# jaxsonpd/air_rs

Hardware: AMD Instinct MI355X
Metric: IQ Msamples/s (decoded Mode-S msgs/s alongside), 2 MSPS i8 stream (higher is better)
Workload: dtype i8; 1 GPU; 2 MSPS i8 IQ, 1 GiB synthetic buffer per GPU, fused magnitude+preamble/DF17 gate+PPM+CRC-24; samples_per_gpu=536870912, bytes_per_gpu=1073741824, channels=1

## Files before the change

air_rs_amd/csrc/adsb_kernels.hip:

```cpp
#include <hip/hip_ext.h>
#include <utility>
#include <cstdlib>

#include "adsb_kernels.h"
#include "adsb_synth.h"

namespace adsbk {

typedef unsigned int u32x4 __attribute__((ext_vector_type(4)));
typedef unsigned short u16x2 __attribute__((ext_vector_type(2)));

__device__ __forceinline__ uint32_t pkmin(uint32_t a, uint32_t b)
{
    u16x2 r = __builtin_elementwise_min(__builtin_bit_cast(u16x2, a), __builtin_bit_cast(u16x2, b));
    return __builtin_bit_cast(uint32_t, r);
}
__device__ __forceinline__ uint32_t pkmax(uint32_t a, uint32_t b)
{
    u16x2 r = __builtin_elementwise_max(__builtin_bit_cast(u16x2, a), __builtin_bit_cast(u16x2, b));
    return __builtin_bit_cast(uint32_t, r);
}
typedef _Float16 f16x2 __attribute__((ext_vector_type(2)));
template <bool F16> __device__ __forceinline__ uint32_t pkmax3(uint32_t a, uint32_t b, uint32_t c)
{
// ... 65 lines not shown
    float f[8];
#pragma unroll
    for (int k = 0; k < 4; k += 2) {
        f32x2 ta = {__builtin_bit_cast(float, a[k]), __builtin_bit_cast(float, a[k + 1])};
        f32x2 tb = {__builtin_bit_cast(float, b[k]), __builtin_bit_cast(float, b[k + 1])};
        f32x2 te = ta - (f32x2){8388607.5f, 8388607.5f};
        f32x2 to = __builtin_elementwise_fma(ta, (f32x2){-0x1.fffffep-1f, -0x1.fffffep-1f}, tb);
        f[2 * k] = te.x;
        f[2 * k + 1] = to.x;
        f[2 * k + 2] = te.y;
        f[2 * k + 3] = to.y;
    }
    float r[8];
#pragma unroll
    for (int k = 0; k < 8; ++k) {
        r[k] = __builtin_amdgcn_sqrtf(f[k]);
        if (MAGMODE == 2) r[k] -= 0.5f;
    }
    lo = __builtin_amdgcn_cvt_pk_u8_f32(r[0], 0, 0u);
    lo = __builtin_amdgcn_cvt_pk_u8_f32(r[1], 1, lo);
    lo = __builtin_amdgcn_cvt_pk_u8_f32(r[2], 2, lo);
    lo = __builtin_amdgcn_cvt_pk_u8_f32(r[3], 3, lo);
    hi = __builtin_amdgcn_cvt_pk_u8_f32(r[4], 0, 0u);
    hi = __builtin_amdgcn_cvt_pk_u8_f32(r[5], 1, hi);
    hi = __builtin_amdgcn_cvt_pk_u8_f32(r[6], 2, hi);
    hi = __builtin_amdgcn_cvt_pk_u8_f32(r[7], 3, hi);
}

__device__ __forceinline__ uint32_t mag_i16_fix(uint32_t r, uint32_t n)
{
    return r - ((__umul24(r, r) > n) ? 1u : 0u);
}
__device__ __forceinline__ uint32_t mag_i16(uint32_t iq)
{
    uint32_t n, r;
    asm("v_dot2_i32_i16 %0, %2, %2, 0\n\t"
        "s_nop 2\n\t"
        "v_cvt_f32_u32 %1, %0\n\t"
        "v_sqrt_f32 %1, %1\n\t"
        "s_nop 0\n\t"
        "v_cvt_rpi_i32_f32 %1, %1"
        : "=&v"(n), "=&v"(r)
        : "v"(iq));
    return mag_i16_fix(r, n);
}
__device__ __forceinline__ void mags4_i16(u32x4 v, uint32_t &lo, uint32_t &hi)
{
    uint32_t n0, n1, n2, n3, r0, r1, r2, r3;
    asm("v_dot2_i32_i16 %0, %8, %8, 0\n\t"
        "v_dot2_i32_i16 %1, %9, %9, 0\n\t"
        "v_dot2_i32_i16 %2, %10, %10, 0\n\t"
        "v_dot2_i32_i16 %3, %11, %11, 0\n\t"
        "s_nop 2\n\t"
        "v_cvt_f32_u32 %4, %0\n\t"
        "v_cvt_f32_u32 %5, %1\n\t"
        "v_cvt_f32_u32 %6, %2\n\t"
        "v_cvt_f32_u32 %7, %3\n\t"
        "v_sqrt_f32 %4, %4\n\t"
        "v_sqrt_f32 %5, %5\n\t"
        "v_sqrt_f32 %6, %6\n\t"
        "v_sqrt_f32 %7, %7\n\t"
        "v_cvt_rpi_i32_f32 %4, %4\n\t"
        "v_cvt_rpi_i32_f32 %5, %5\n\t"
        "v_cvt_rpi_i32_f32 %6, %6\n\t"
        "s_nop 0\n\t"
        "v_cvt_rpi_i32_f32 %7, %7\n\t"
        "s_nop 0"
        : "=&v"(n0), "=&v"(n1), "=&v"(n2), "=&v"(n3), "=&v"(r0), "=&v"(r1), "=&v"(r2), "=&v"(r3)
        : "v"(v.x), "v"(v.y), "v"(v.z), "v"(v.w));
    lo = __builtin_amdgcn_perm(mag_i16_fix(r1, n1), mag_i16_fix(r0, n0), 0x05040100u);
    hi = __builtin_amdgcn_perm(mag_i16_fix(r3, n3), mag_i16_fix(r2, n2), 0x05040100u);
}

__global__ void probe_cvt_kernel(uint32_t *out)
{
    if (threadIdx.x != 0) return;
    float a = 0.75f, b = 2.5f, c = 180.9986f;
    asm volatile("" : "+v"(a), "+v"(b), "+v"(c));
    uint32_t r0 = __builtin_amdgcn_cvt_pk_u8_f32(a, 0, 0u);
    r0 = __builtin_amdgcn_cvt_pk_u8_f32(b, 1, r0);
    r0 = __builtin_amdgcn_cvt_pk_u8_f32(c, 2, r0);
    out[0] = r0;
    __builtin_amdgcn_s_setreg((1 | (0 << 6) | ((2 - 1) << 11)), 3);
    asm volatile("" : "+v"(a), "+v"(b), "+v"(c));
    uint32_t r1 = __builtin_amdgcn_cvt_pk_u8_f32(a, 0, 0u);
    r1 = __builtin_amdgcn_cvt_pk_u8_f32(b, 1, r1);
    r1 = __builtin_amdgcn_cvt_pk_u8_f32(c, 2, r1);
    out[1] = r1;
    __builtin_amdgcn_s_setreg((1 | (0 << 6) | ((2 - 1) << 11)), 0);
    out[2] = 0xC0DEu;
    out[3] = 0;
}

hipError_t probe_cvt(hipStream_t s, uint32_t *dev_scratch4, uint32_t host_out[4])
{
    hipLaunchKernelGGL(probe_cvt_kernel, dim3(1), dim3(64), 0, s, dev_scratch4);
    hipError_t e = hipGetLastError();
    if (e != hipSuccess) return e;
    e = hipMemcpyAsync(host_out, dev_scratch4, 16, hipMemcpyDeviceToHost, s);
    if (e != hipSuccess) return e;
    return hipStreamSynchronize(s);
}

template <int ST> struct MagT;
template <> struct MagT<ADSB_SAMPLE_I8> { typedef uint8_t type; };
template <> struct MagT<ADSB_SAMPLE_I16> { typedef uint16_t type; };

template <int ST> struct Lds {
    typedef typename MagT<ST>::type mag_t;
    static constexpr int kMagBytes = (TileCfg<ST>::kMagT * (int)sizeof(mag_t) + 15) & ~15;
    static constexpr int kOffCand = kMagBytes;
    static constexpr int kOffList = kOffCand + 2 * kThreads * 4 * ((TileCfg<ST>::kRunT + 31) / 32);
    static constexpr int kOffMisc = kOffList + kListCap * 2;
    static constexpr int kTotal = kOffMisc + 64;
};

template <int ST>
__device__ __forceinline__ uint32_t pair_at(const uint32_t *ra, const uint32_t *rb, int k)
{
    if (ST == ADSB_SAMPLE_I8) {
        const uint32_t sel = 0x0C000C00u | (uint32_t)(k & 3) | ((uint32_t)(4 + (k & 3)) << 16);
        return __builtin_amdgcn_perm(rb[k >> 2], ra[k >> 2], sel);
    } else {
        const uint32_t sel = (k & 1) ? 0x07060302u : 0x05040100u;
        return __builtin_amdgcn_perm(rb[k >> 1], ra[k >> 1], sel);
    }
}

template <int ST>
__device__ __forceinline__ uint32_t pair_at_cold(const uint32_t *ra, const uint32_t *rb, int k)
{
    if (ST == ADSB_SAMPLE_I8) {
        const uint32_t sel = 0x0C000C00u | (uint32_t)(4 + (k & 3)) | ((uint32_t)(k & 3) << 16);
        return __builtin_amdgcn_perm(ra[k >> 2], rb[k >> 2], sel);
    } else {
        const uint32_t sel = (k & 1) ? 0x03020706u : 0x01000504u;
        return __builtin_amdgcn_perm(ra[k >> 1], rb[k >> 1], sel);
    }
}

#define ADSB_DPP(v, ctrl) ((uint32_t)__builtin_amdgcn_update_dpp(0, (int)(v), (ctrl), 0xF, 0xF, true))
__device__ __forceinline__ uint32_t row16_xor(uint32_t v)
{
    v ^= ADSB_DPP(v, 0xB1);
    v ^= ADSB_DPP(v, 0x4E);
    v ^= ADSB_DPP(v, 0x141);
    v ^= ADSB_DPP(v, 0x140);
    return v;
}

template <int ST>
__device__ __forceinline__ uint32_t slice_byte(const typename MagT<ST>::type *mag, const uint32_t off, const uint32_t lb)
{
    uint32_t byte = 0;
    if (ST == ADSB_SAMPLE_I16) {
        const typename MagT<ST>::type *mp = mag + off + 16 + 16 * lb;
#pragma unroll
        for (int k = 0; k < 8; ++k)
            byte |= (((uint32_t)mp[2 * k + 1] - (uint32_t)mp[2 * k]) >> 31) << (7 - k);
    } else {
        const uint32_t pidx = off + 16 + 16 * lb;
        const uint32_t *mw = reinterpret_cast<const uint32_t *>(mag) + (pidx >> 2);
        const uint32_t sh = pidx & 3;
        const uint32_t d0 = mw[0], d1 = mw[1], d2 = mw[2], d3 = mw[3], d4 = mw[4];
        uint32_t w[4] = {__builtin_amdgcn_alignbyte(d1, d0, sh), __builtin_amdgcn_alignbyte(d2, d1, sh),
                         __builtin_amdgcn_alignbyte(d3, d2, sh), __builtin_amdgcn_alignbyte(d4, d3, sh)};
        uint64_t m0, m1, m2, m3, m4, m5, m6, m7;
        asm("v_cmp_gt_u32_sdwa %1, %9, %9 src0_sel:BYTE_0 src1_sel:BYTE_1\n\t"
            "v_cmp_gt_u32_sdwa %2, %9, %9 src0_sel:BYTE_2 src1_sel:BYTE_3\n\t"
            "v_cmp_gt_u32_sdwa %3, %10, %10 src0_sel:BYTE_0 src1_sel:BYTE_1\n\t"
            "v_cmp_gt_u32_sdwa %4, %10, %10 src0_sel:BYTE_2 src1_sel:BYTE_3\n\t"
            "v_cmp_gt_u32_sdwa %5, %11, %11 src0_sel:BYTE_0 src1_sel:BYTE_1\n\t"
            "v_cmp_gt_u32_sdwa %6, %11, %11 src0_sel:BYTE_2 src1_sel:BYTE_3\n\t"
            "v_cmp_gt_u32_sdwa %7, %12, %12 src0_sel:BYTE_0 src1_sel:BYTE_1\n\t"
            "v_cmp_gt_u32_sdwa %8, %12, %12 src0_sel:BYTE_2 src1_sel:BYTE_3\n\t"
            "v_addc_co_u32_e64 %0, vcc, %0, %0, %1\n\t"
            "v_addc_co_u32_e64 %0, vcc, %0, %0, %2\n\t"
            "v_addc_co_u32_e64 %0, vcc, %0, %0, %3\n\t"
            "v_addc_co_u32_e64 %0, vcc, %0, %0, %4\n\t"
            "v_addc_co_u32_e64 %0, vcc, %0, %0, %5\n\t"
            "v_addc_co_u32_e64 %0, vcc, %0, %0, %6\n\t"
            "v_addc_co_u32_e64 %0, vcc, %0, %0, %7\n\t"
            "v_addc_co_u32_e64 %0, vcc, %0, %0, %8"
            : "+v"(byte), "=&s"(m0), "=&s"(m1), "=&s"(m2), "=&s"(m3), "=&s"(m4), "=&s"(m5), "=&s"(m6), "=&s"(m7)
            : "v"(w[0]), "v"(w[1]), "v"(w[2]), "v"(w[3])
            : "vcc");
    }
    return byte;
}

__device__ __forceinline__ bool count_candidate(const bool have, const uint32_t byte, const uint32_t l, const uint32_t lane)
{
    const uint32_t lb = l < 14 ? l : 13;
    uint32_t s = 0;
    const uint32_t *sy = kSyn.v + 8 * lb;
    const int sb = (int)(l < 14 ? byte : 0u);
#pragma unroll
    for (int k = 0; k < 8; ++k) s ^= sy[k] & (uint32_t)((sb << (24 + k)) >> 31);
    s = row16_xor(s);
    int found = -1;
    if (s != 0 && l < 11) {
#pragma unroll
        for (int k = 0; k < 8; ++k) found = (sy[k] == s) ? k : found;
    }
    const unsigned long long fm = __ballot(found >= 0);
    const uint32_t gbits = (uint32_t)(fm >> (lane & 48u)) & 0xFFFFu;
    return have && (s == 0 || gbits != 0);
}

struct TilePos {
    uint32_t ch;
    uint64_t sample0;
    uint32_t n_valid;
};
template <int TILE = kTile>
__device__ __forceinline__ TilePos tile_pos(const DemodArgs &p, uint32_t tile)
{
    TilePos t;
    t.ch = tile / p.tiles_per_channel;
    const uint32_t tch = tile - t.ch * p.tiles_per_channel;
    t.sample0 = (uint64_t)tch * TILE;
    const uint64_t left = (p.n_samples - kWindow) - t.sample0;
    t.n_valid = left < (uint64_t)TILE ? (uint32_t)left : (uint32_t)TILE;
    return t;
}

template <int BPS, int MAG = kMag>
__device__ __forceinline__ __amdgpu_buffer_rsrc_t tile_rsrc(const DemodArgs &p, const TilePos &t, bool live = true)
{
    const char *base = (const char *)p.iq + ((uint64_t)t.ch * p.channel_stride + t.sample0) * BPS;
    const uint64_t remain = (p.n_samples - t.sample0) * BPS;
    const uint32_t nrec = remain > (uint64_t)(MAG * BPS) ? (uint32_t)(MAG * BPS) : (uint32_t)remain;
    return __builtin_amdgcn_make_buffer_rsrc((void *)base, 0, live ? (int)nrec : 0, 0x00020000);
}

#ifndef ADSB_TILE_STAMPS
#define ADSB_TILE_STAMPS 0
#endif
#if ADSB_TILE_STAMPS
#define TSTAMP(k)                                                                                              \
    do {                                                                                                       \
        if ((tid & 63u) == 0 && (wave == 0 || wave == 3)) {                                                    \
            __builtin_amdgcn_sched_barrier(0);                                                                 \
            const unsigned long long now_ = __builtin_amdgcn_s_memtime();                                      \
            if ((k) >= 0) ts_seg[(k)] = (uint32_t)(now_ - ts_prev);                                            \
            ts_prev = now_;                                                                                    \
            __builtin_amdgcn_sched_barrier(0);                                                                 \
        }                                                                                                      \
    } while (0)
#else
#define TSTAMP(k) do { } while (0)
#endif

#ifndef ADSB_AB_KERNELS
#define ADSB_AB_KERNELS 0
#endif
bool ab_kernels_built() { return ADSB_AB_KERNELS != 0; }

template <int RUN, int NT>
__device__ __forceinline__ void gate_collect(uint32_t *candA, uint32_t *candB, uint16_t *list, uint32_t *count,
                                             const uint32_t tid, const uint32_t n_valid)
{
    constexpr int WPR = (RUN + 31) / 32;
    const uint32_t sa = tid * RUN, sb = (tid + NT) * RUN;
    const uint32_t va = n_valid > sa ? (n_valid - sa) : 0u, vb = n_valid > sb ? (n_valid - sb) : 0u;
    uint32_t words[2 * WPR];
    uint32_t nz = 0, c = 0;
#pragma unroll
    for (int k = 0; k < WPR; ++k) {
        words[k] = candA[k];
        words[WPR + k] = candB[k];
    }
    if (n_valid < (uint32_t)(2 * NT * RUN)) {
#pragma unroll
        for (int k = 0; k < WPR; ++k) {
            const uint32_t la = va > 32u * k ? va - 32u * k : 0u, lb = vb > 32u * k ? vb - 32u * k : 0u;
            words[k] &= la >= 32u ? 0xFFFFFFFFu : ((1u << la) - 1u);
            words[WPR + k] &= lb >= 32u ? 0xFFFFFFFFu : ((1u << lb) - 1u);
            candA[k] = words[k];
            candB[k] = words[WPR + k];
        }
    }
#pragma unroll
    for (int k = 0; k < 2 * WPR; ++k) {
        nz |= words[k];
        c += __builtin_popcount(words[k]);
    }
    if (nz) {
        uint32_t pos = atomicAdd(count, c);
#pragma unroll
        for (int k = 0; k < 2 * WPR; ++k) {
            uint32_t bits = words[k];
            const uint32_t base = (k < WPR ? sa : sb) + (k % WPR) * 32;
            while (bits) {
                const uint32_t b = __builtin_ctz(bits);
                bits &= bits - 1;
                if (pos < (uint32_t)kSparseCap) list[pos] = (uint16_t)(base + b);
                ++pos;
            }
        }
    }
}

template <int ST, int RUN, int NT, bool F16OK = (ST == ADSB_SAMPLE_I8)>
__device__ __forceinline__ void gate_phase(const typename MagT<ST>::type *mag, uint32_t *cand, uint16_t *list,
                                           uint32_t *count, const uint32_t tid, const uint32_t n_valid)
{
    static_assert(RUN == 16 || RUN == 32 || RUN == 64, "1 or 2 bitmap words per run");
    constexpr int WPR = (RUN + 31) / 32;
    constexpr int SPG = 16 / (int)sizeof(typename MagT<ST>::type);
    uint32_t *candA = cand + WPR * tid, *candB = cand + WPR * (tid + NT);
#pragma unroll
    for (int k = 0; k < WPR; ++k) candA[k] = candB[k] = 0u;
    constexpr int kGran = (RUN + 26 + SPG - 1) / SPG + 1;
    const u32x4 *ga = reinterpret_cast<const u32x4 *>(mag + tid * RUN);
    const u32x4 *gb = reinterpret_cast<const u32x4 *>(mag + (tid + NT) * RUN);
    uint32_t ra[kGran * 4], rb[kGran * 4];
    constexpr int kAhead = 48 / SPG;
#pragma unroll
    for (int g = 0; g < kAhead; ++g) {
        u32x4 a = ga[g], b = gb[g];
        ra[4 * g] = a.x; ra[4 * g + 1] = a.y; ra[4 * g + 2] = a.z; ra[4 * g + 3] = a.w;
        rb[4 * g] = b.x; rb[4 * g + 1] = b.y; rb[4 * g + 2] = b.z; rb[4 * g + 3] = b.w;
    }

    uint32_t N[RUN + 26], H2[RUN + 8], W3[RUN + 16], F[RUN + 9];
#pragma unroll
    for (int k = 0; k < 25; ++k) N[k] = pair_at<ST>(ra, rb, k);
#pragma unroll
    for (int j = 0; j < 7; ++j) H2[j] = pkmin(N[j], N[j + 2]);
#pragma unroll
    for (int j = 3; j < 13; ++j) W3[j] = pkmax3<F16OK>(N[j], N[j + 1], N[j + 2]);
#pragma unroll
    for (int j = 1; j < 8; ++j) F[j] = pkmax3<F16OK>(N[j], W3[j + 2], N[j + 5]);

#pragma unroll
    for (int o = 0; o < RUN; ++o) {
        if (o % SPG == 0) {
            const int g = o / SPG + kAhead;
            if (g * SPG < RUN + 26) {
                u32x4 a = ga[g], b = gb[g];
                ra[4 * g] = a.x; ra[4 * g + 1] = a.y; ra[4 * g + 2] = a.z; ra[4 * g + 3] = a.w;
                rb[4 * g] = b.x; rb[4 * g + 1] = b.y; rb[4 * g + 2] = b.z; rb[4 * g + 3] = b.w;
            }
        }
        N[o + 25] = pair_at<ST>(ra, rb, o + 25);
        W3[o + 13] = pkmax3<F16OK>(N[o + 13], N[o + 14], N[o + 15]);
        F[o + 8] = pkmax3<F16OK>(N[o + 8], W3[o + 10], N[o + 13]);
        const uint32_t lo = pkmax3<F16OK>(F[o + 1], F[o + 8], W3[o + 13]);
        H2[o + 7] = pkmin(N[o + 7], N[o + 9]);
        const uint32_t hi = pkmin(H2[o], H2[o + 7]);
        const bool pa = (uint16_t)hi >= (uint16_t)lo;
        const bool pb = (hi >> 16) >= (lo >> 16);
        if (__builtin_expect(__builtin_amdgcn_ballot_w64(pa | pb) != 0, 0)) {
            const uint32_t dh = pkmin3<F16OK>(pkmin3<F16OK>(N[o + 16], N[o + 19], N[o + 21]), N[o + 23], N[o + 24]);
            const uint32_t dl = pkmax3<F16OK>(pkmax3<F16OK>(N[o + 17], N[o + 18], N[o + 20]), N[o + 22], N[o + 25]);
            const bool da = (uint16_t)dh >= (uint16_t)dl;
            const bool db = (dh >> 16) >= (dl >> 16);
            uint32_t bit = 1u << (o & 31);
            asm("" : "+v"(bit));
            if (pa & da) atomicOr(candA + (o >> 5), bit);
            if (pb & db) atomicOr(candB + (o >> 5), bit);
        }
    }
    gate_collect<RUN, NT>(candA, candB, list, count, tid, n_valid);
}

#ifndef ADSB_LOAD_AUX
#define ADSB_LOAD_AUX 2
#endif
template <int ST> struct P1 {
    static constexpr int kSPL = ST == ADSB_SAMPLE_I8 ? 8 : 4;
    static constexpr int kIters = (TileCfg<ST>::kMagT + kThreads * kSPL - 1) / (kThreads * kSPL);
};

template <int ST>
__device__ __forceinline__ void issue_tile_loads(const DemodArgs &p, const TilePos &tp, bool live, uint32_t tid,
                                                 u32x4 (&raw)[P1<ST>::kIters])
{
    constexpr int BPS = (ST == ADSB_SAMPLE_I8) ? 2 : 4;
    __amdgpu_buffer_rsrc_t rsrc = tile_rsrc<BPS, TileCfg<ST>::kMagT>(p, tp, live);
    const uint32_t wave_s0 = __builtin_amdgcn_readfirstlane(tid & ~63u) * P1<ST>::kSPL;
#pragma unroll
    for (int it = 0; it < P1<ST>::kIters; ++it)
        if ((uint32_t)it * (kThreads * P1<ST>::kSPL) + wave_s0 < (uint32_t)TileCfg<ST>::kMagT)
            raw[it] = __builtin_amdgcn_raw_buffer_load_b128(rsrc, tid * 16, (uint32_t)it * (kThreads * 16), ADSB_LOAD_AUX);
}

template <int ST, int MAGMODE>
__device__ __forceinline__ bool magnitudes_to_lds(const u32x4 (&raw)[P1<ST>::kIters], typename MagT<ST>::type *mag, uint32_t tid)
{
    uint32_t mx = 0;
    const uint32_t wave_s0 = __builtin_amdgcn_readfirstlane(tid & ~63u) * P1<ST>::kSPL;
#pragma unroll
    for (int it = 0; it < P1<ST>::kIters; ++it) {
        if ((uint32_t)it * (kThreads * P1<ST>::kSPL) + wave_s0 < (uint32_t)TileCfg<ST>::kMagT) {
            const uint32_t s = (uint32_t)it * (kThreads * P1<ST>::kSPL) + tid * P1<ST>::kSPL;
            uint32_t lo, hi;
            if (ST == ADSB_SAMPLE_I8) mags8_i8<MAGMODE>(raw[it], lo, hi);
            else {
                mags4_i16(raw[it], lo, hi);
                mx = pkmax(mx, pkmax(lo, hi));
            }
            if (s < (uint32_t)TileCfg<ST>::kMagT) *reinterpret_cast<uint2 *>(mag + s) = make_uint2(lo, hi);
        }
    }
    return ST == ADSB_SAMPLE_I16 && __builtin_amdgcn_ballot_w64(((mx & 0xFFFFu) >= 0x7C00u) || ((mx >> 16) >= 0x7C00u)) != 0;
}

__device__ __forceinline__ void clear_launch_flags(const DemodArgs &p, const bool first, const uint32_t tid)
{
    if (tid == 0 && first) {
        p.hdr->retry = 0;
        if (p.count_groups) {
            p.hdr->flags = 0;
            if (p.hdr_pub) p.hdr_pub[2] = 0;
        }
    }
}
__device__ __forceinline__ void tile_prologue(const DemodArgs &p, const bool first, uint32_t *misc, const uint32_t tid)
{
    clear_launch_flags(p, first, tid);
    if (tid == 0) {
        misc[8] = 0;
        misc[12] = 0;
    }
}


__device__ __forceinline__ void put_record(adsb_frame *slot, const uint64_t o64, const uint32_t byte, const uint32_t l)
{
    unsigned char *rec = reinterpret_cast<unsigned char *>(slot);
    if (l < 14) rec[8 + l] = (unsigned char)byte;
    else reinterpret_cast<uint32_t *>(rec)[l - 14] = l == 14 ? (uint32_t)o64 : (uint32_t)(o64 >> 32);
}

__device__ __forceinline__ void write_seg(const DemodArgs &p, const uint32_t tile, const uint32_t base_slot, const uint32_t cand,
                                          const uint32_t valid)
{
    Seg e;
    e.base = base_slot;
    e.cand = cand;
    e.valid = valid;
    e.decoded = base_slot == kNoBase ? 1u : 0u;
    p.seg[tile] = e;
}

constexpr uint32_t kCountBitmap = 0xFFFFFFFFu;
struct NoRecheck {
    __device__ __forceinline__ void operator()(uint16_t *, uint32_t) const {}
};
template <int TILE, int BITS, class SLICER, class RECHECK = NoRecheck>
__device__ __forceinline__ void hand_over(const DemodArgs &p, const uint32_t tile, const uint64_t sample0, uint32_t total,
                                          const uint32_t *cand, uint16_t *list, uint32_t *misc, const uint32_t tid,
                                          const uint32_t lane, const uint32_t wave, SLICER slicer, RECHECK recheck = RECHECK())
{
    const bool dense = total > (uint32_t)kSparseCap;
    u32x4 cw = {0, 0, 0, 0};
    uint32_t cnt = 0, my_first = 0;
    if (dense) {
        if (4 * tid < (uint32_t)(TILE / BITS)) cw = reinterpret_cast<const u32x4 *>(cand)[tid];
        cnt = __builtin_popcount(cw.x) + __builtin_popcount(cw.y) + __builtin_popcount(cw.z) +
              __builtin_popcount(cw.w);
        uint32_t incl = cnt;
#pragma unroll
        for (int d = 1; d < 64; d <<= 1) {
            uint32_t t = __shfl_up(incl, d, 64);
            if ((int)lane >= d) incl += t;
        }
        if (lane == 63) misc[wave] = incl;
        __syncthreads();
        uint32_t wbase = 0;
        total = 0;
#pragma unroll
        for (int w = 0; w < kThreads / 64; ++w) {
            uint32_t t = misc[w];
            wbase += (w < (int)wave) ? t : 0u;
            total += t;
        }
        my_first = wbase + incl - cnt;
    }

    const bool simple = !dense && total <= kQuota;
    const uint64_t abs0 = sample0 + p.offset_base;
    uint32_t base_slot = tile * kQuota;
    const uint32_t g = tid >> 4, l = tid & 15;
    auto slice_round = [&](uint32_t slot0, uint32_t ncl) {
        for (uint32_t r = 0; r < ncl; r += kThreads / 16) {
            if (r + 4 * wave >= ncl) break;
            const uint32_t ci = r + g;
            const bool have = ci < ncl;
            const uint32_t off = have ? list[ci] : 0u;
            bool dropped;
            const uint32_t byte = slicer(have, off, l, dropped);
            if (have) put_record(p.slots + (size_t)slot0 + ci, dropped ? ~0ull : abs0 + off, byte, l);
        }
    };
    if (simple) {
        slice_round(base_slot, total);
    } else {
        if (tid == 0) {
            const unsigned long long b64 = atomicAdd(&p.hdr->alloc, (unsigned long long)total);
            misc[9] = (!p.pool_off && b64 + total <= (unsigned long long)p.cap_slots) ? p.pool_first + (uint32_t)b64 : kNoBase;
        }
        __syncthreads();
        base_slot = misc[9];
        for (uint32_t chunk = 0; chunk < total; chunk += kListCap) {
            if (dense && cnt) {
                uint32_t idx = my_first;
                const uint32_t words[4] = {cw.x, cw.y, cw.z, cw.w};
#pragma unroll
                for (int k = 0; k < 4; ++k) {
                    uint32_t bits = words[k];
                    while (bits) {
                        const uint32_t b = __builtin_ctz(bits);
                        bits &= bits - 1;
                        if (idx >= chunk && idx < chunk + kListCap)
                            list[idx - chunk] = (uint16_t)((4 * tid + k) * BITS + b);
                        ++idx;
                    }
                }
            }
            __syncthreads();
            const uint32_t ncl = (total - chunk) < (uint32_t)kListCap ? (total - chunk) : (uint32_t)kListCap;
            if (dense) recheck(list, ncl);
            if (base_slot != kNoBase) {
                slice_round(base_slot + chunk, ncl);
            } else {
                for (uint32_t r = 0; r < ncl; r += kThreads / 16) {
                    if (r + 4 * wave >= ncl) break;
                    const uint32_t ci = r + g;
                    const bool have = ci < ncl;
                    const uint32_t off = have ? list[ci] : 0u;
                    bool dropped;
                    const uint32_t byte = slicer(have, off, l, dropped);
                    const bool valid = count_candidate(have && !dropped, byte, l, lane);
                    if (valid && l == 0) atomicAdd(&misc[8], 1u);
                }
            }
            __syncthreads();
        }
    }
    if (tid == 0) write_seg(p, tile, base_slot, total, misc[8]);
}

#ifndef ADSB_SCAN_WAVES
#define ADSB_SCAN_WAVES 4
#endif
template <int ST, int MAGMODE>
__device__ __forceinline__ void scan_tile(const DemodArgs &p, const uint32_t tile, const bool first, unsigned char *smem)
{
    typedef Lds<ST> L;
    typedef TileCfg<ST> TC;
    typedef typename L::mag_t mag_t;
    static_assert(kThreads / 64 <= 4, "misc[4 + wave] must stay below misc[8]");

    mag_t *mag = reinterpret_cast<mag_t *>(smem);
    uint32_t *cand = reinterpret_cast<uint32_t *>(smem + L::kOffCand);
    uint16_t *list = reinterpret_cast<uint16_t *>(smem + L::kOffList);
    uint32_t *misc = reinterpret_cast<uint32_t *>(smem + L::kOffMisc);

    const uint32_t tid = threadIdx.x;
    const uint32_t lane = tid & 63, wave = tid >> 6;

    if (MAGMODE == 1) __builtin_amdgcn_s_setreg((1 | (0 << 6) | ((2 - 1) << 11)), 3);
#if ADSB_TILE_STAMPS
    unsigned long long ts_prev = 0;
    uint32_t ts_seg[9] = {0, 0, 0, 0, 0, 0, 0, 0, 0};
    ts_seg[7] = (uint32_t)__builtin_amdgcn_s_memrealtime();
    TSTAMP(-1);
    ts_seg[8] = (uint32_t)ts_prev;
#endif
    {
        const TilePos tp = tile_pos<TC::kTileT>(p, tile);
        const uint64_t sample0 = tp.sample0;
        const uint32_t n_valid = tp.n_valid;
        u32x4 raw[P1<ST>::kIters];
        issue_tile_loads<ST>(p, tp, true, tid, raw);
        TSTAMP(0);
        tile_prologue(p, first, misc, tid);
#if ADSB_TILE_STAMPS
        asm volatile("s_waitcnt vmcnt(0)" ::: "memory");
        TSTAMP(6);
#endif
        const bool wave_big = magnitudes_to_lds<ST, MAGMODE>(raw, mag, tid);
        if (ST == ADSB_SAMPLE_I16 && lane == 0) misc[4 + wave] = wave_big ? 1u : 0u;
        TSTAMP(1);
        __syncthreads();
        TSTAMP(2);

        if constexpr (ST == ADSB_SAMPLE_I16) {
            uint32_t any_big = 0;
#pragma unroll
            for (int w = 0; w < kThreads / 64; ++w) any_big |= misc[4 + w];
            const bool big = any_big != 0;
            if (!big) gate_phase<ST, TC::kRunT, kThreads, true>(mag, cand, list, &misc[12], tid, n_valid);
            else gate_phase<ST, TC::kRunT, kThreads, false>(mag, cand, list, &misc[12], tid, n_valid);
        } else {
            gate_phase<ST, TC::kRunT, kThreads>(mag, cand, list, &misc[12], tid, n_valid);
        }
        TSTAMP(3);
        __syncthreads();
        TSTAMP(4);

        constexpr int kBitsPerWord = TC::kRunT < 32 ? TC::kRunT : 32;
        hand_over<TC::kTileT, kBitsPerWord>(p, tile, sample0, misc[12], cand, list, misc, tid, lane, wave,
                                            [=](const bool, const uint32_t off, const uint32_t l, bool &dropped) {
                                                dropped = false;
                                                return slice_byte<ST>(mag, off, l < 14 ? l : 13);
                                            });
        TSTAMP(5);
#if ADSB_TILE_STAMPS
        if ((tid & 63u) == 0 && (wave == 0 || wave == 3)) {
            uint32_t *dst = reinterpret_cast<uint32_t *>(p.stamps) + (size_t)tile * 16 + (wave ? 8 : 0);
#pragma unroll
            for (int k = 0; k < 8; ++k) dst[k] = ts_seg[k];
            if (wave) dst[6] = ts_seg[8];
        }
#endif
    }
    if (MAGMODE == 1) __builtin_amdgcn_s_setreg((1 | (0 << 6) | ((2 - 1) << 11)), 0);
}

#ifndef ADSB_XCD_MAP
#define ADSB_XCD_MAP 1
#endif
__device__ __forceinline__ uint32_t tile_of_workgroup(uint32_t b, uint32_t n)
{
#if ADSB_XCD_MAP
    const uint32_t q = n >> 3, r = n & 7u, x = b & 7u, j = b >> 3;
    return x * q + (x < r ? x : r) + j;
#else
    (void)n;
    return b;
#endif
}

template <int ST, int MAGMODE>
__global__ __launch_bounds__(kThreads, ST == ADSB_SAMPLE_I8 ? 8 : ADSB_SCAN_WAVES) void demod_tiles(DemodArgs p)
{
    __shared__ __attribute__((aligned(16))) unsigned char smem[Lds<ST>::kTotal];
    scan_tile<ST, MAGMODE>(p, p.tile_first + tile_of_workgroup(blockIdx.x, p.tile_count), blockIdx.x == 0, smem);
}

struct CrcTable {
    uint32_t v[256];
};
constexpr CrcTable make_crc_table()
{
    CrcTable t{};
    for (uint32_t i = 0; i < 256; ++i) {
        uint32_t r = i << 16;
        for (int k = 0; k < 8; ++k) {
            r <<= 1;
            if (r & 0x1000000u) r ^= 0x1FFF409u;
        }
        t.v[i] = r & 0xFFFFFFu;
    }
    return t;
}
__constant__ CrcTable kCrcTab = make_crc_table();
struct SynSorted {
    uint32_t v[128];
};
constexpr SynSorted make_syn_sorted()
{
    SynSorted t{};
    SynTable sy = make_syn();
    for (int j = 0; j < 128; ++j) t.v[j] = j < 88 ? ((sy.v[j] << 7) | (uint32_t)j) : 0xFFFFFFFFu;
    for (int i = 1; i < 128; ++i) {
        uint32_t x = t.v[i];
        int k = i - 1;
        while (k >= 0 && t.v[k] > x) {
            t.v[k + 1] = t.v[k];
            --k;
        }
        t.v[k + 1] = x;
    }
    return t;
}
__constant__ SynSorted kSynSorted = make_syn_sorted();

constexpr int kFinTiles = 32;
constexpr int kFinThreads = 256;
constexpr int kFinFan = 64;
constexpr int kFinFlat = 1024;
constexpr uint32_t kLbReady = 1u;
constexpr uint32_t kLbSpinLimit = 1u << 21;

__device__ __forceinline__ bool finish_record(uint32_t (&w)[6], const bool have, const uint32_t *crc_tab, const uint32_t *syn_sorted)
{
    uint32_t crc = 0;
#pragma unroll
    for (int i = 0; i < 11; ++i) {
        const uint32_t b = (w[2 + (i >> 2)] >> (8 * (i & 3))) & 0xFFu;
        crc = ((crc << 8) ^ crc_tab[((crc >> 16) ^ b) & 0xFFu]) & 0xFFFFFFu;
    }
    const uint32_t rx = ((w[4] >> 24) << 16) | ((w[5] & 0xFFu) << 8) | ((w[5] >> 8) & 0xFFu);
    const uint32_t sm = crc ^ rx;
    uint32_t pos = 0;
#pragma unroll
    for (int step = 64; step >= 1; step >>= 1)
        pos += ((syn_sorted[pos + step - 1] >> 7) < sm) ? (uint32_t)step : 0u;
    const uint32_t hit = syn_sorted[pos];
    const bool found = sm != 0 && (hit >> 7) == sm;
    const bool valid = have && (sm == 0 || found);
    const bool fix = valid && sm != 0;
    const uint32_t fixed = fix ? (hit & 0x7Fu) : 0xFFu;
    const uint32_t status = valid ? (sm == 0 ? 0u : 1u) : 0xFFu;
    const uint32_t bi = 8u + ((hit & 0x7Fu) >> 3);
    const uint32_t flip = fix ? ((0x80u >> (hit & 7u)) << (8u * (bi & 3u))) : 0u;
    const uint32_t wi = bi >> 2;
    w[2] ^= wi == 2 ? flip : 0u;
    w[3] ^= wi == 3 ? flip : 0u;
    w[4] ^= wi == 4 ? flip : 0u;
    w[5] = (w[5] & 0xFFFFu) | (status << 16) | (fixed << 24);
    return valid;
}


template <int N> __device__ __forceinline__ uint32_t row_ror(uint32_t v)
{
    return (uint32_t)__builtin_amdgcn_update_dpp(0, (int)v, 0x120 + N , 0xF, 0xF, true);
}
__device__ __forceinline__ uint32_t row_rank(uint32_t key)
{
    uint32_t below = 0;
#define ADSB_RANK_STEP(N) below += row_ror<N>(key) < key ? 1u : 0u;
    ADSB_RANK_STEP(1) ADSB_RANK_STEP(2) ADSB_RANK_STEP(3) ADSB_RANK_STEP(4) ADSB_RANK_STEP(5)
    ADSB_RANK_STEP(6) ADSB_RANK_STEP(7) ADSB_RANK_STEP(8) ADSB_RANK_STEP(9) ADSB_RANK_STEP(10)
    ADSB_RANK_STEP(11) ADSB_RANK_STEP(12) ADSB_RANK_STEP(13) ADSB_RANK_STEP(14) ADSB_RANK_STEP(15)
#undef ADSB_RANK_STEP
    return below;
}

__device__ __forceinline__ void store_record(adsb_frame *dst, const uint32_t (&w)[6])
{
    uint2 *d = reinterpret_cast<uint2 *>(dst);
#pragma unroll
    for (int k = 0; k < 3; ++k) d[k] = make_uint2(w[2 * k], w[2 * k + 1]);
}
__device__ __forceinline__ void load_record(const adsb_frame *src, uint32_t (&w)[6])
{
    const uint2 *s2 = reinterpret_cast<const uint2 *>(src);
#pragma unroll
    for (int k = 0; k < 3; ++k) {
        const uint2 v = s2[k];
        w[2 * k] = v.x;
        w[2 * k + 1] = v.y;
    }
}

__device__ __forceinline__ uint32_t finish_big_tile(const FinishArgs &a, const Seg &e, const uint32_t *crc_tab,
                                                    const uint32_t *syn_sorted, uint32_t lane)
{
    uint32_t n_good = 0;
    for (uint32_t chunk = 0; chunk < e.cand; chunk += 64) {
        const uint32_t nc = (e.cand - chunk) < 64u ? (e.cand - chunk) : 64u;
        uint32_t w[6] = {0xFFFFFFFFu, 0xFFFFFFFFu, 0, 0, 0, 0};
        if (lane < nc) load_record(a.slots + (size_t)e.base + chunk + lane, w);
        const bool valid = finish_record(w, lane < nc && w[1] != 0xFFFFFFFFu, crc_tab, syn_sorted);
        uint32_t slot = lane;
        if (e.cand <= (uint32_t)kSparseCap) {
            const bool rec = lane < nc && w[1] != 0xFFFFFFFFu;
            const unsigned long long rm = __ballot(rec);
            const uint32_t ref = rm ? (uint32_t)__builtin_amdgcn_readlane((int)w[0], (int)__builtin_ctzll(rm)) : 0u;
            const int32_t mine = rec ? (int32_t)(w[0] - ref) : (int32_t)(0x40000000u + lane);
            uint32_t below = 0;
            for (uint32_t k = 0; k < nc; ++k) {
                const int32_t other = (int32_t)__builtin_amdgcn_readlane((int)mine, (int)k);
                below += other < mine ? 1u : 0u;
            }
            slot = below;
        }
        if (lane < nc) store_record(a.slots + (size_t)e.base + chunk + slot, w);
        n_good += (uint32_t)__builtin_popcountll(__ballot(valid));
    }
    return n_good;
}

constexpr int kFinLdsWords = 256 + 128 + 2 * kFinTiles;
template <bool PUB_ATOMIC = true>
__device__ __forceinline__ void finish_block(const FinishArgs &a, const uint32_t blk, const uint32_t n_blk, uint32_t *lds)
{
    uint32_t *crc_tab = lds, *syn_sorted = lds + 256;
    uint32_t *counts = lds + 384;
    uint32_t *tpos = lds + 384 + kFinTiles;
    const uint32_t tid = threadIdx.x, lane = tid & 63, wave = tid >> 6, g = lane >> 4, sub = lane & 15;
    const uint32_t tile0 = a.tile_first + blk * kFinTiles, t_end = a.tile_first + a.tile_count;

    Seg e[2];
    uint32_t w[2][6], rank[2];
    bool valid[2], small_[2];
#pragma unroll
    for (int p = 0; p < 2; ++p) {
        const uint32_t idx = wave * 8 + p * 4 + g, tile = tile0 + idx;
        e[p].base = kNoBase; e[p].cand = 0; e[p].valid = 0; e[p].decoded = 1;
        w[p][0] = w[p][1] = 0xFFFFFFFFu;
        w[p][2] = w[p][3] = w[p][4] = w[p][5] = 0;
        if (tile < t_end) {
            e[p] = a.seg[tile];
            load_record(a.slots + (size_t)tile * kQuota + sub, w[p]);
        }
    }
    for (uint32_t i = tid; i < 256 + 128; i += kFinThreads) {
        if (i < 256) crc_tab[i] = kCrcTab.v[i];
        else syn_sorted[i - 256] = kSynSorted.v[i - 256];
    }
    __syncthreads();
#pragma unroll
    for (int p = 0; p < 2; ++p) {
        const bool live = e[p].cand != 0 && e[p].base != kNoBase && !e[p].decoded;
        small_[p] = live && e[p].cand <= 16u;
        if (!(small_[p] && sub < e[p].cand)) {
            w[p][0] = w[p][1] = 0xFFFFFFFFu;
            w[p][2] = w[p][3] = w[p][4] = w[p][5] = 0;
        }
    }
#pragma unroll
    for (int p = 0; p < 2; ++p) {
        const uint32_t idx = wave * 8 + p * 4 + g;
        valid[p] = finish_record(w[p], small_[p] && sub < e[p].cand && w[p][1] != 0xFFFFFFFFu, crc_tab, syn_sorted);
        const uint32_t recs = (uint32_t)(__ballot(w[p][1] != 0xFFFFFFFFu) >> (16u * g)) & 0xFFFFu;
        const uint32_t ref = (uint32_t)__shfl((int)w[p][0], (int)((lane & 48u) + (recs ? (uint32_t)__builtin_ctz(recs) : 0u)), 64);
        const uint32_t key = valid[p] ? ((w[p][0] - ref + 0x8000u) & 0xFFFFu) : 0x10000u;
        rank[p] = row_rank(key);
        const uint32_t cnt = (uint32_t)__builtin_popcount((uint32_t)(__ballot(valid[p]) >> (16u * g)) & 0xFFFFu);
        if (sub == 0) counts[idx] = small_[p] ? cnt : (e[p].decoded ? e[p].valid : 0u);
    }
    uint32_t big_mask = 0;
#pragma unroll
    for (int p = 0; p < 2; ++p) {
        const bool big = e[p].cand > 16u && e[p].base != kNoBase && !e[p].decoded;
        const unsigned long long m = __ballot(big && sub == 0);
        big_mask |= (uint32_t)(((m >> 0) & 1u) | ((m >> 15) & 2u) | ((m >> 30) & 4u) | ((m >> 45) & 8u)) << (4 * p);
    }
    for (uint32_t left = big_mask; left; left &= left - 1) {
        const uint32_t i = (uint32_t)__builtin_ctz(left), idx = wave * 8 + i;
        const Seg eb = a.seg[tile0 + idx];
        const uint32_t n_good = finish_big_tile(a, eb, crc_tab, syn_sorted, lane);
        if (lane == 0) counts[idx] = n_good;
    }
    __syncthreads();

// ... 487 lines not shown
```

Before: 2.757 million Msamples/s.

## Append gate candidates inline and add early-return fast path in hand_over

The gate phase now appends each surviving candidate offset straight to the LDS list with a returning ds_add, instead of running a separate gate_collect pass that popcounts the bitmap and expands it. The bitmap is still set, and its tail past n_valid is masked. hand_over gains an early-return path for tiles with at most kQuota candidates, and makes total and wave wave-uniform via readfirstlane. The aim is to cut the post-gate collect pass, its atomics and barriers in the common sparse case. The cost is serialized per-candidate LDS atomics with waitcnt inside the hot loop, plus list ordering that now depends on atomic order.

```diff
diff --git a/air_rs_amd/csrc/adsb_kernels.hip b/air_rs_amd/csrc/adsb_kernels.hip
--- a/air_rs_amd/csrc/adsb_kernels.hip
+++ b/air_rs_amd/csrc/adsb_kernels.hip
@@ -391,6 +391,30 @@
     }
 }
 
+__device__ __forceinline__ void gate_append(uint16_t *list, uint32_t *count, const uint32_t off, const uint32_t n_valid)
+{
+    if (off < n_valid) {
+        uint32_t pos = (uint32_t)(uintptr_t)(__attribute__((address_space(3))) uint32_t *)count;
+        const uint32_t one = 1u;
+        asm volatile("ds_add_rtn_u32 %0, %0, %1\n\ts_waitcnt lgkmcnt(0)" : "+v"(pos) : "v"(one) : "memory");
+        if (pos < (uint32_t)kSparseCap) list[pos] = (uint16_t)off;
+    }
+}
+
+template <int RUN, int NT>
+__device__ __forceinline__ void gate_mask_tail(uint32_t *candA, uint32_t *candB, const uint32_t tid, const uint32_t n_valid)
+{
+    constexpr int WPR = (RUN + 31) / 32;
+    const uint32_t sa = tid * RUN, sb = (tid + NT) * RUN;
+    const uint32_t va = n_valid > sa ? (n_valid - sa) : 0u, vb = n_valid > sb ? (n_valid - sb) : 0u;
+#pragma unroll
+    for (int k = 0; k < WPR; ++k) {
+        const uint32_t la = va > 32u * k ? va - 32u * k : 0u, lb = vb > 32u * k ? vb - 32u * k : 0u;
+        candA[k] &= la >= 32u ? 0xFFFFFFFFu : ((1u << la) - 1u);
+        candB[k] &= lb >= 32u ? 0xFFFFFFFFu : ((1u << lb) - 1u);
+    }
+}
+
 template <int ST, int RUN, int NT, bool F16OK = (ST == ADSB_SAMPLE_I8)>
 __device__ __forceinline__ void gate_phase(const typename MagT<ST>::type *mag, uint32_t *cand, uint16_t *list,
                                            uint32_t *count, const uint32_t tid, const uint32_t n_valid)
@@ -441,18 +465,26 @@
         const uint32_t hi = pkmin(H2[o], H2[o + 7]);
         const bool pa = (uint16_t)hi >= (uint16_t)lo;
         const bool pb = (hi >> 16) >= (lo >> 16);
+        const unsigned long long mpa = __builtin_amdgcn_ballot_w64(pa), mpb = __builtin_amdgcn_ballot_w64(pb);
         if (__builtin_expect(__builtin_amdgcn_ballot_w64(pa | pb) != 0, 0)) {
             const uint32_t dh = pkmin3<F16OK>(pkmin3<F16OK>(N[o + 16], N[o + 19], N[o + 21]), N[o + 23], N[o + 24]);
             const uint32_t dl = pkmax3<F16OK>(pkmax3<F16OK>(N[o + 17], N[o + 18], N[o + 20]), N[o + 22], N[o + 25]);
-            const bool da = (uint16_t)dh >= (uint16_t)dl;
-            const bool db = (dh >> 16) >= (dl >> 16);
-            uint32_t bit = 1u << (o & 31);
-            asm("" : "+v"(bit));
-            if (pa & da) atomicOr(candA + (o >> 5), bit);
-            if (pb & db) atomicOr(candB + (o >> 5), bit);
-        }
-    }
-    gate_collect<RUN, NT>(candA, candB, list, count, tid, n_valid);
+            const unsigned long long sva = mpa & __builtin_amdgcn_ballot_w64((uint16_t)dh >= (uint16_t)dl);
+            const unsigned long long svb = mpb & __builtin_amdgcn_ballot_w64((dh >> 16) >= (dl >> 16));
+            if (__builtin_expect((sva | svb) != 0, 0)) {
+                const bool va = __builtin_amdgcn_inverse_ballot_w64(sva), vb = __builtin_amdgcn_inverse_ballot_w64(svb);
+                uint32_t bit = 1u << (o & 31);
+                asm("" : "+v"(bit));
+                if (va) atomicOr(candA + (o >> 5), bit);
+                if (vb) atomicOr(candB + (o >> 5), bit);
+                uint32_t t = tid;
+                asm("" : "+v"(t));
+                if (va) gate_append(list, count, t * RUN + o, n_valid);
+                if (vb) gate_append(list, count, (t + NT) * RUN + o, n_valid);
+            }
+        }
+    }
+    if (n_valid < (uint32_t)(2 * NT * RUN)) gate_mask_tail<RUN, NT>(candA, candB, tid, n_valid);
 }
 
 #ifndef ADSB_LOAD_AUX
@@ -542,8 +574,29 @@
 template <int TILE, int BITS, class SLICER, class RECHECK = NoRecheck>
 __device__ __forceinline__ void hand_over(const DemodArgs &p, const uint32_t tile, const uint64_t sample0, uint32_t total,
                                           const uint32_t *cand, uint16_t *list, uint32_t *misc, const uint32_t tid,
-                                          const uint32_t lane, const uint32_t wave, SLICER slicer, RECHECK recheck = RECHECK())
-{
+                                          const uint32_t lane, uint32_t wave, SLICER slicer, RECHECK recheck = RECHECK())
+{
+    total = __builtin_amdgcn_readfirstlane(total);
+    wave = __builtin_amdgcn_readfirstlane(wave);
+    const uint64_t abs0 = sample0 + p.offset_base;
+    const uint32_t g = tid >> 4, l = tid & 15;
+    auto slice_round = [&](uint32_t slot0, uint32_t ncl) {
+        for (uint32_t r = 0; r + 4 * wave < ncl; r += kThreads / 16) {
+            const uint32_t ci = r + g;
+            const bool have = ci < ncl;
+            const uint32_t off = have ? list[ci] : 0u;
+            bool dropped;
+            const uint32_t byte = slicer(have, off, l, dropped);
+            if (have) put_record(p.slots + (size_t)slot0 + ci, dropped ? ~0ull : abs0 + off, byte, l);
+        }
+    };
+
+    if (total <= kQuota) {
+        if (tid == 0) write_seg(p, tile, tile * kQuota, total, misc[8]);
+        slice_round(tile * kQuota, total);
+        return;
+    }
+
     const bool dense = total > (uint32_t)kSparseCap;
     u32x4 cw = {0, 0, 0, 0};
     uint32_t cnt = 0, my_first = 0;
@@ -568,67 +621,48 @@
             total += t;
         }
         my_first = wbase + incl - cnt;
-    }
-
-    const bool simple = !dense && total <= kQuota;
-    const uint64_t abs0 = sample0 + p.offset_base;
-    uint32_t base_slot = tile * kQuota;
-    const uint32_t g = tid >> 4, l = tid & 15;
-    auto slice_round = [&](uint32_t slot0, uint32_t ncl) {
-        for (uint32_t r = 0; r < ncl; r += kThreads / 16) {
-            if (r + 4 * wave >= ncl) break;
-            const uint32_t ci = r + g;
-            const bool have = ci < ncl;
-            const uint32_t off = have ? list[ci] : 0u;
-            bool dropped;
-            const uint32_t byte = slicer(have, off, l, dropped);
-            if (have) put_record(p.slots + (size_t)slot0 + ci, dropped ? ~0ull : abs0 + off, byte, l);
-        }
-    };
-    if (simple) {
-        slice_round(base_slot, total);
-    } else {
-        if (tid == 0) {
-            const unsigned long long b64 = atomicAdd(&p.hdr->alloc, (unsigned long long)total);
-            misc[9] = (!p.pool_off && b64 + total <= (unsigned long long)p.cap_slots) ? p.pool_first + (uint32_t)b64 : kNoBase;
-        }
-        __syncthreads();
-        base_slot = misc[9];
-        for (uint32_t chunk = 0; chunk < total; chunk += kListCap) {
-            if (dense && cnt) {
-                uint32_t idx = my_first;
-                const uint32_t words[4] = {cw.x, cw.y, cw.z, cw.w};
-#pragma unroll
-                for (int k = 0; k < 4; ++k) {
-                    uint32_t bits = words[k];
-                    while (bits) {
-                        const uint32_t b = __builtin_ctz(bits);
-                        bits &= bits - 1;
-                        if (idx >= chunk && idx < chunk + kListCap)
-                            list[idx - chunk] = (uint16_t)((4 * tid + k) * BITS + b);
-                        ++idx;
-                    }
+        total = __builtin_amdgcn_readfirstlane(total);
+    }
+
+    if (tid == 0) {
+        const unsigned long long b64 = atomicAdd(&p.hdr->alloc, (unsigned long long)total);
+        misc[9] = (!p.pool_off && b64 + total <= (unsigned long long)p.cap_slots) ? p.pool_first + (uint32_t)b64 : kNoBase;
+    }
+    __syncthreads();
+    const uint32_t base_slot = misc[9];
+    for (uint32_t chunk = 0; chunk < total; chunk += kListCap) {
+        if (dense && cnt) {
+            uint32_t idx = my_first;
+            const uint32_t words[4] = {cw.x, cw.y, cw.z, cw.w};
+#pragma unroll
+            for (int k = 0; k < 4; ++k) {
+                uint32_t bits = words[k];
+                while (bits) {
+                    const uint32_t b = __builtin_ctz(bits);
+                    bits &= bits - 1;
+                    if (idx >= chunk && idx < chunk + kListCap)
+                        list[idx - chunk] = (uint16_t)((4 * tid + k) * BITS + b);
+                    ++idx;
                 }
             }
-            __syncthreads();
-            const uint32_t ncl = (total - chunk) < (uint32_t)kListCap ? (total - chunk) : (uint32_t)kListCap;
-            if (dense) recheck(list, ncl);
-            if (base_slot != kNoBase) {
-                slice_round(base_slot + chunk, ncl);
-            } else {
-                for (uint32_t r = 0; r < ncl; r += kThreads / 16) {
-                    if (r + 4 * wave >= ncl) break;
-                    const uint32_t ci = r + g;
-                    const bool have = ci < ncl;
-                    const uint32_t off = have ? list[ci] : 0u;
-                    bool dropped;
-                    const uint32_t byte = slicer(have, off, l, dropped);
-                    const bool valid = count_candidate(have && !dropped, byte, l, lane);
-                    if (valid && l == 0) atomicAdd(&misc[8], 1u);
-                }
+        }
+        __syncthreads();
+        const uint32_t ncl = (total - chunk) < (uint32_t)kListCap ? (total - chunk) : (uint32_t)kListCap;
+        if (dense) recheck(list, ncl);
+        if (base_slot != kNoBase) {
+            slice_round(base_slot + chunk, ncl);
+        } else {
+            for (uint32_t r = 0; r + 4 * wave < ncl; r += kThreads / 16) {
+                const uint32_t ci = r + g;
+                const bool have = ci < ncl;
+                const uint32_t off = have ? list[ci] : 0u;
+                bool dropped;
+                const uint32_t byte = slicer(have, off, l, dropped);
+                const bool valid = count_candidate(have && !dropped, byte, l, lane);
+                if (valid && l == 0) atomicAdd(&misc[8], 1u);
             }
-            __syncthreads();
-        }
+        }
+        __syncthreads();
     }
     if (tid == 0) write_seg(p, tile, base_slot, total, misc[8]);
 }
```

New measurement: 2.815 million Msamples/s, median of 6. 2.1% higher.
